# m-schuetz/SimLOD

Hardware: AMD Instinct MI355X
Metric: M points/sec inserted into octree (raster M samples/s @1080p under 'raster') (higher is better)
Workload: dtype f32+u32 (fp32 quantise/project, fp64 pixel coordinate, integer octree/atomics); 1 GPU; Morro Bay 36M stand-in (BASELINE config 2): 36000000 16 B points, fractal terrain, 36 x 1M ring batches resident in HBM, reset + 2.0 kernel_construct launches per step; raster 1920x1080; points_per_gpu=36000000, record_order=shuffled, parallelism=one global cube, level-3 cells dealt to 1 rank(s) by point count

## Files before the change

### simlod_amd/csrc/construct.hip

```cpp
#include <mutex>
#include "simlod_device.hpp"
#include "simlod_hip.h"
#include "simlod_internal.hpp"

namespace simlod {
namespace build {

#include "construct_state.inc"
#include "construct_begin.inc"
#include "construct_count.inc"
#include "construct_expand.inc"
#include "construct_voxelize.inc"
#include "construct_insert.inc"

static_assert(offsetof(Ctl, groupMax) == 44 && offsetof(Ctl, expandNs) + 4 * sizeof(uint64_t) == 184, "Ctl.groupMax at byte 44, Ctl.expandNs[4] at byte 184");

static inline uint64_t align_up(uint64_t v, uint64_t a) { return (v + a - 1) / a * a; }

static constexpr uint64_t ACCT_SPILL_FLOOR = 3500000;
bool layout_construct(BuildArgs& a, uint64_t capacity, bool coalesce, uint32_t groupLimit = SIMLOD_MAX_BATCHES_PER_LAUNCH, uint32_t exactGroup = 1) {
	a.dirCap = 2 * a.nodeCapacity + 65536;
	a.acct = exactGroup > 1u ? 1u : 0u;
	uint64_t off = 4096;
	a.offQueue = off;    off += align_up((uint64_t)CHUNK_QUEUE_CAPACITY * 8, 256);
	a.offSlots = off;    off += align_up((uint64_t)2 * SLOT_CAP * sizeof(SlotRec), 256);
	a.offHist = off;     off += align_up(((uint64_t)SLOT_CAP * HIST_BINS + HIST_EXTRA_WORDS) * 4, 256);
	a.offMap = off;      off += align_up((uint64_t)SLOT_CAP * HIST_BINS * 4, 256);
	a.offHistB = off;    off += align_up((uint64_t)(a.acct ? SLOT_CAP : 0u) * HIST_BINS * exactGroup * 4, 256);
	a.clearCap = 65536;
	a.offClear = off;    off += align_up((uint64_t)2 * a.clearCap * 8, 256);
	a.offTouched = off;  off += align_up((uint64_t)a.nodeCapacity * 4, 256);
	a.crossCap = 16384;
	a.offCross = off;    off += align_up((uint64_t)a.crossCap * 4, 256);
	a.offSplitTag = off; off += align_up((uint64_t)a.nodeCapacity * 8, 256);
	a.offRetryTag = off; off += align_up((uint64_t)a.nodeCapacity * 4, 256);
	a.offTouchTag = off; off += align_up((uint64_t)a.nodeCapacity * 4, 256);
	a.offStartOf = off;  off += align_up((uint64_t)a.nodeCapacity * 8, 256);
	a.offCntB = off;     off += align_up((uint64_t)(a.acct ? a.nodeCapacity : 0u) * exactGroup * 4, 256);
	a.hashCap = 1u << 17;
	a.offHashDir = off;  off += align_up((uint64_t)a.hashCap * sizeof(DirEntry), 256);
	a.offParent = off;   off += align_up((uint64_t)a.nodeCapacity * 4, 256);
	a.offNodeDir = off;  off += align_up((uint64_t)a.nodeCapacity * sizeof(NodeDir), 256);
	a.offChunkDir = off; off += align_up(2ull * a.dirCap * 8, 256);
	a.offLeafChunks = off; off += (uint64_t)a.nodeCapacity * LEAF_ROW_BYTES;
	a.offPaths = off; off += align_up((uint64_t)a.nodeCapacity * PATH_WORDS * 8, 256);
	a.offTop = off;   off += align_up((uint64_t)TOP_CELLS * 4, 256);
	a.offKid = off;   off += align_up((uint64_t)a.nodeCapacity * 4, 256);
	a.voxItemCap = min(a.nodeCapacity + 2u * VOX_BIG_ITEMS, 1u << 20);
	a.offVoxItems = off; off += align_up(2ull * a.voxItemCap * sizeof(VoxItem), 256);
	const uint64_t perBatch = (uint64_t)SIMLOD_MAX_BATCH_SIZE * 4;
	const uint64_t fixedWork = ((uint64_t)SPILLING_CAPACITY + a.nodeCapacity / 8) * 32;
	a.groupMax = 1; a.groupCap = SIMLOD_MAX_BATCH_SIZE;
	if (capacity < off + 2 * perBatch + fixedWork + 4096 + 25ull * 65536) { a.spilledCap = 0; a.scratchBytes = off + 2 * perBatch + fixedWork; return false; }
	const uint64_t freeBytes = capacity - off - fixedWork - 4096;
	if (coalesce) a.groupMax = (uint32_t)std::max<uint64_t>(1, std::min<uint64_t>(std::min<uint32_t>(groupLimit, SIMLOD_MAX_BATCHES_PER_LAUNCH), freeBytes / (2 * perBatch + 20ull * SIMLOD_MAX_BATCH_SIZE)));
	if (a.acct) {
		if (freeBytes < 2ull * exactGroup * perBatch + 512 + ACCT_SPILL_FLOOR * 20032 / 1000) return false;
		a.groupMax = exactGroup;
	}
	a.groupCap = a.groupMax * SIMLOD_MAX_BATCH_SIZE;
	uint64_t cap = (freeBytes - 2ull * a.groupMax * perBatch - 512) * 1000 / (20 * 1000 + 32);
	if (cap > 0x7fffffffull - a.groupCap) cap = 0x7fffffffull - a.groupCap;
	a.spilledCap = (uint32_t)cap;
	a.workCap = a.spilledCap / SIMLOD_POINTS_PER_CHUNK + a.nodeCapacity / 8 + SPILLING_CAPACITY;
	a.offWork = off;     off += align_up((uint64_t)a.workCap * 32, 256);
	a.leafOfStride = align_up((uint64_t)a.groupCap * 4, 256) / 4;
	a.offLeafOf = off;   off += 2 * a.leafOfStride * 4 + align_up((uint64_t)a.spilledCap * 4, 256);
	a.offSpilled = off;  off += (uint64_t)a.spilledCap * 16;
	a.scratchBytes = off;
	return off <= capacity;
}

}
struct SideStream {
	hipStream_t stream;
	hipEvent_t expanded[SIMLOD_MAX_BATCHES_PER_LAUNCH], inserted[SIMLOD_MAX_BATCHES_PER_LAUNCH], tailDone;
	std::mutex enqueue;
};
// ... 139 lines not shown
```

### simlod_amd/csrc/construct_begin.inc

```

__device__ __forceinline__ bool stamp_is_stale(const BuildArgs& a, const Ctl* ctl) {
	const uint32_t first = a.stats->batchletIndex;
	return ctl->tableMagic != TABLE_MAGIC || ctl->tableBatch != first || ctl->tableNodes != (uint64_t)a.nodes || ctl->tablePers != (uint64_t)a.pers ||
	       ctl->tableLayout != layout_signature(a) || ctl->tableSig != table_signature(a.stats) ||
	       (first >= 0x80000u && (first & 0x7ffffu) < SIMLOD_MAX_BATCHES_PER_LAUNCH);
}

__device__ __forceinline__ SimlodChunk*& tail_of(SimlodChunk* head) { return *reinterpret_cast<SimlodChunk**>(&head->size); }

__device__ void rebuild_side_tables(const BuildArgs& a, bool irregular) {
	const uint64_t first = (uint64_t)blockIdx.x * TPB + threadIdx.x, stride = (uint64_t)gridDim.x * TPB;
	{
		uint4* w = reinterpret_cast<uint4*>(a.mom + a.offSplitTag);
		const uint64_t n = (a.offParent - a.offSplitTag) / 16;
		for (uint64_t i = first; i < n; i += stride) w[i] = make_uint4(0, 0, 0, 0);
	}
	const uint32_t numNodes = min(a.stats->numNodes, a.nodeCapacity);
	uint32_t* parentOf = at<uint32_t>(a, a.offParent);
	for (uint64_t i = first; i < TOP_CELLS; i += stride) {
		const uint32_t s = (uint32_t)SIMLOD_MAX_DEPTH - TOP_LEVEL;
		const uint32_t X = ((uint32_t)i >> (2u * TOP_LEVEL)) << s, Y = (((uint32_t)i >> TOP_LEVEL) & (TOP_SIDE - 1u)) << s, Z = ((uint32_t)i & (TOP_SIDE - 1u)) << s;
		uint32_t cur = 0, level = 0;
		while (level < TOP_LEVEL) {
			const SimlodNode* c = a.nodes[cur].children[child_index(X, Y, Z, (int)level)];
// ... 11 lines not shown
			if (c != nullptr) parentOf[(uint32_t)(c - a.nodes)] = (uint32_t)i;
		}
		{
			const SimlodNode* c0 = n->children[0];
			uint32_t word = 0u, some = 0u;
			bool regular = c0 != nullptr;
#pragma unroll
			for (int k = 0; k < 8; k++) {
				const SimlodNode* c = n->children[k];
				if (c != nullptr) some++;
				if (c == nullptr || c != c0 + k) regular = false;
				else if (node_is_leaf(c)) word |= 1u << (KID_LEAF_SHIFT + (uint32_t)k);
			}
			at<uint32_t>(a, a.offKid)[i] = some == 0u ? 0u : regular && !irregular ? (word | (uint32_t)(c0 - a.nodes)) : KID_IRREGULAR;
		}
		uint8_t* const table = a.mom + a.offLeafChunks;
		const bool leaf = node_is_leaf(n);
		SimlodChunk* const head = leaf ? n->points : n->voxelChunks;
		const uint32_t inList = ((leaf ? n->numPoints : n->numVoxelsStored) + SIMLOD_POINTS_PER_CHUNK - 1) / SIMLOD_POINTS_PER_CHUNK;
		SimlodChunk* c = head;
		for (uint32_t k = 0; c != nullptr && k < max(inList, 1u); k++) {
			if (k < LEAF_SLOTS) leaf_row_set(table, a.pers, i, k, c);
			if (k + 1u == inList) tail_of(head) = c;
			c = c->next;
		}
		if (leaf && n->voxelChunks != nullptr) {
			const uint32_t inVox = (n->numVoxelsStored + SIMLOD_POINTS_PER_CHUNK - 1) / SIMLOD_POINTS_PER_CHUNK;
			SimlodChunk* v = n->voxelChunks;
			for (uint32_t k = 0; v != nullptr && k < max(inVox, 1u); k++) {
				if (k + 1u >= inVox) { tail_of(n->voxelChunks) = v; break; }
				v = v->next;
			}
		}
		unsigned long long* rec = at<unsigned long long>(a, a.offPaths) + i * PATH_WORDS;
		const uint32_t L = min(n->level, PATH_WORDS - 1u), s = (uint32_t)SIMLOD_MAX_DEPTH - L;
		const uint32_t X = n->X << s, Y = n->Y << s, Z = n->Z << s;
		uint32_t cur = 0, l = 0;
		for (; l < L; l++) {
			const SimlodNode* anc = a.nodes + cur;
			rec[L - 1u - l] = path_pack(a.pers, cur, anc->level, anc->grid);
			const SimlodNode* c = anc->children[child_index(X, Y, Z, (int)l)];
			if (c == nullptr) break;
			cur = (uint32_t)(c - a.nodes);
		}
		rec[L] = 0;
	}
}

__global__ __launch_bounds__(TPB) void k_begin(BuildArgs a, uint32_t momentaryTooSmall, uint32_t batchLimit, uint32_t debugFlags, uint32_t budgetUs, uint32_t groupMax) {
	Ctl* ctl = ctl_of(a);
	const bool stale = momentaryTooSmall != 0u || (debugFlags & 4u) != 0u || stamp_is_stale(a, ctl);
	if (threadIdx.x == 0 && blockIdx.x == 0) {
		const uint32_t fatal = a.stats->dbg & (SIMLOD_ERR_BARRIER_TIMEOUT | SIMLOD_ERR_DIRECTORY_FULL | SIMLOD_ERR_IMPORT | SIMLOD_ERR_IMPORT_GRID);
		ctl->errors = momentaryTooSmall ? SIMLOD_ERR_MOMENTARY_TOO_SMALL : 0u;
		ctl->stop = (momentaryTooSmall || fatal) ? 1u : 0u;
		ctl->abortBatch = 0;
		ctl->processed = 0;
		ctl->consumed = 0;
		ctl->pointsTaken = a.stats->numPointsProcessed;
		ctl->groupMax = groupMax;
		ctl->debugFlags = debugFlags;
		ctl->budgetUs = budgetUs != 0u ? budgetUs : (uint32_t)(SIMLOD_MAX_PROCESSING_MS * 1000.0f);
		ctl->startNs = wall_ns();
		*a.frameStart = ctl->startNs;
		const uint32_t uploaded = __hip_atomic_load(a.numBatchesUploaded, __ATOMIC_RELAXED, __HIP_MEMORY_SCOPE_AGENT);
		const uint32_t first = a.stats->batchletIndex;
		uint32_t n = uploaded - first;
		if ((int32_t)n < 0) n = 0;
		if (n > SIMLOD_MAX_BATCHES_PER_LAUNCH) n = SIMLOD_MAX_BATCHES_PER_LAUNCH;
		if (n > batchLimit) n = batchLimit;
		ctl->uploaded = uploaded;
		ctl->firstBatch = first;
		ctl->numBatches = n;
		for (int i = 0; i < 8; i++) ctl->statCounters[i] = 0;
		ctl->rebuildLeafChunks = stale ? 1u : 0u;
		if (momentaryTooSmall != 0u) ctl->tableMagic = 0;
		for (uint32_t i = 0; i < BATCH_COPIES; i++) ctl->batch[i].active = 0;
		for (uint32_t i = 0; i < SIMLOD_MAX_BATCHES_PER_LAUNCH; i++) { ctl->voxT[i][0] = ~0ull; ctl->voxT[i][1] = 0; ctl->voxT[i][2] = 0; }
// ... 5 lines not shown
```

### simlod_amd/csrc/construct_expand.inc

```

static constexpr uint32_t VTPB = 1024;
#ifndef VOX_SPT_N
#define VOX_SPT_N 8
#endif
static constexpr uint32_t VOX_SPT = VOX_SPT_N;
static constexpr uint32_t VOX_PIECE = VTPB * VOX_SPT;
static constexpr uint32_t VOX_BIG_ITEMS = 65536;
static constexpr uint32_t VOX_SMALL = 512;
static constexpr uint32_t VOX_SMALL_PIECE = 128;
static constexpr uint32_t LDS_LEVELS = 7;
static constexpr uint32_t CUBE_WORDS = 8192 + 1024 + 256 + 64 + 16 + 4 + 4;
struct VoxItem { uint32_t leaf, s0, s1, ptBase, ptFirst; };
__device__ __forceinline__ VoxItem* vox_items(const BuildArgs& a, const BatchCtl* bc) { return at<VoxItem>(a, a.offVoxItems) + (uint64_t)(bc->ordinal & 1u) * a.voxItemCap; }

#ifndef ALLOC_WAVES_N
#define ALLOC_WAVES_N 10
#endif
static constexpr uint32_t ALLOC_WAVES = ALLOC_WAVES_N, ALLOC_LEAVES = 64 * ALLOC_WAVES;
struct AllocRec {
	uint32_t node, existing, additional, fromPool;
	uint32_t dirNew, prefix;
	unsigned long long firstIdx, mem;
	SimlodChunk* head; SimlodChunk* tail;
};
// ... 373 lines not shown
			}
		}
		if (histHere) {
			__syncthreads();
			for (uint32_t e = threadIdx.x; e < HT_CAP; e += ETPB) {
				const uint32_t key = sh.keys[e];
				if (key != TBL_EMPTY) hist_flush(a, key, sh.vals[e], acct);
			}
			if (timer) { t1 = wall_ns(); ctl->expandNs[0] += t1 - t0; t0 = t1; }
			if (!grid_barrier(&bc->barrierCount, generation, gridDim.x)) { if (threadIdx.x == 0) panic(ctl, SIMLOD_ERR_BARRIER_TIMEOUT); return; }
			if (timer) { t1 = wall_ns(); ctl->expandNs[1] += t1 - t0; t0 = t1; }
		}

		Phase pd(ctl, blockIdx.x == 0);
		for (uint32_t s = sb + blockIdx.x; s < se; s += gridDim.x) {
			uint32_t t = threadIdx.x;
			asm volatile("" : "+v"(t));
			uint64_t before[6] = {0, 0, 0, 0, 0, 0};
			if (pd.on) for (uint32_t k = 0; k < 6u; k++) before[k] = ctl->phaseNs[32u + k];
			const uint32_t myBin = t < HIST_BINS ? hist_sum(hist, (uint64_t)s * HIST_BINS + t) : 0u;
			const SlotRec rec = slots[s];
			if (rec.node == NONE) { if (t == 0u) atomicAdd(&bc->decided, 1u); continue; }
			const uint32_t L = rec.node, l = rec.level;
			const uint32_t K = min(3u, (uint32_t)SIMLOD_MAX_DEPTH - l);
			__syncthreads();
			uint32_t* const B3 = sh.keys; uint32_t* const B2 = B3 + HIST_BINS * GBS; uint32_t* const B1 = B2 + 64u * GBS;
			uint32_t binTotal = myBin;
			if (acct && t < HIST_BINS) {
				const uint32_t* hb = at<const uint32_t>(a, a.offHistB) + ((uint64_t)s * HIST_BINS + t) * GBS;
				for (uint32_t k = 0; k < GB; k++) { const uint32_t r = hb[k]; B3[t * GBS + k] = r; binTotal += r; }
			}
			if (t < HIST_BINS) sh.bins[t] = binTotal;
			if (t < SIMLOD_MAX_BATCHES_PER_LAUNCH) { sh.accD[t] = 0; sh.accF[t] = 0; }
			if (t < PATH_WORDS) sh.pathL[t] = t + 1 < PATH_WORDS ? paths[(uint64_t)L * PATH_WORDS + t] : 0ull;
			if (t == 64u) { const SimlodNode* nl = a.nodes + L; sh.LX = nl->X; sh.LY = nl->Y; sh.LZ = nl->Z; sh.gridL = nl->grid; }
			if (t >= 96u && t < 116u) sh.nameL[t - 96u] = a.nodes[L].name[t - 96u];
			for (uint32_t i = t; i < LOCAL_NODES; i += ETPB) sh.listed[i] = NONE;
			if (t < 72u) sh.grid[t] = nullptr;
			if (t == 0u) { sh.numFresh = 0; sh.numFill = 0; }
			__syncthreads();
			if (t < 64u) { uint32_t c = 0; for (uint32_t k = 0; k < 8; k++) c += sh.bins[t * 8 + k]; sh.c2[t] = c; }
			__syncthreads();
			if (t < 8u) { uint32_t c = 0; for (uint32_t k = 0; k < 8; k++) c += sh.c2[t * 8 + k]; sh.c1[t] = c; }
			__syncthreads();
			if (t < 64u) {
				bool f1 = false, f2 = false;
				if (trunk_any(a) && l + 1u < TRUNK_LEVELS) {
					const uint32_t LX = sh.LX, LY = sh.LY, LZ = sh.LZ, j = t >> 3, k = t & 7u;
					f1 = t < 8u && trunk_forced(a, l + 1u, 2u * LX + ((t >> 2) & 1u), 2u * LY + ((t >> 1) & 1u), 2u * LZ + (t & 1u));
					f2 = trunk_forced(a, l + 2u, 4u * LX + 2u * ((j >> 2) & 1u) + ((k >> 2) & 1u), 4u * LY + 2u * ((j >> 1) & 1u) + ((k >> 1) & 1u), 4u * LZ + 2u * (j & 1u) + (k & 1u));
				}
				{ const unsigned long long bf1 = __ballot(f1), bf2 = __ballot(f2); if (t == 0u) { sh.forced1 = (uint32_t)bf1 & 0xffu; sh.forced2 = bf2; } }
				const bool s1 = t < 8u && K >= 2u && (sh.c1[t & 7u] > SIMLOD_MAX_POINTS_PER_NODE || f1);
				uint32_t mask1 = (uint32_t)__ballot(s1) & 0xffu;
				const bool s2 = K >= 3u && ((mask1 >> (t >> 3)) & 1u) != 0u && (sh.c2[t] > SIMLOD_MAX_POINTS_PER_NODE || f2);
				unsigned long long mask2 = __ballot(s2);
				uint32_t n1 = (uint32_t)__popc(mask1), n2 = (uint32_t)__popcll(mask2);
				uint32_t extraBase = 0, granted = n1 + n2;
				if (t == 0 && n1 + n2 > 0u) {
					uint32_t noSlot, noSpill;
					if (!reserve(a, ctl, bc, 0u, 8u * (n1 + n2), 0u, noSlot, extraBase, noSpill)) {
						const uint32_t inUse = (uint32_t)(__hip_atomic_load(&bc->reserve, __ATOMIC_RELAXED, __HIP_MEMORY_SCOPE_AGENT) >> 32) & 0xfffffu;
						granted = a.nodeCapacity > inUse ? min((a.nodeCapacity - inUse) / 8u, n1 + n2) : 0u;
						if (granted == 0u || !reserve(a, ctl, bc, 0u, 8u * granted, 0u, noSlot, extraBase, noSpill)) { granted = 0u; extraBase = NONE; }
					}
				}
				extraBase = __shfl(extraBase, 0); granted = __shfl(granted, 0);
// ... 146 lines not shown
				uint32_t oct[3] = {0, 0, 0};
				for (uint32_t k = 0; k < depth; k++) oct[k] = (rel >> (3u * (depth - 1u - k))) & 7u;
				uint32_t X = sh.LX, Y = sh.LY, Z = sh.LZ;
				for (uint32_t k = 0; k < depth; k++) { X = 2u * X + ((oct[k] >> 2) & 1u); Y = 2u * Y + ((oct[k] >> 1) & 1u); Z = 2u * Z + (oct[k] & 1u); }
				const bool split = splits(t);
				const bool nextRound = sh.listed[t] != NONE;
				SimlodNode& c = a.nodes[idx];
				const uint32_t firstChild = !split ? 0u : t < 8u ? sh.base2[t] : sh.base3[t - 8u];
				for (uint32_t k = 0; k < 8; k++) c.children[k] = split ? a.nodes + firstChild + k : nullptr;
				kidOf[idx] = !split ? 0u : irregularKids ? KID_IRREGULAR : firstChild | ((t < 8u ? ~(uint32_t)(mask2 >> (8u * t)) & 0xffu : 0xffu) << KID_LEAF_SHIFT);
				uint32_t counter = countOf(t);
				if (acct) {
					if (depth == 3u) {
						const uint32_t born = sh.splitAt[8u + ((t - 72u) >> 3)];
						uint32_t cThen = 0;
						const uint32_t at = nextRound ? split_time(t, born, false, cThen) : NEVER;
						sh.splitAt[t] = (uint8_t)at; sh.counterAt[t] = cThen;
						leaf_chunks(t, born, at);
					}
					if (sh.splitAt[t] != NEVER) counter = sh.counterAt[t];
				}
				c.counter = counter; c.numPoints = 0;
				c.level = level; c.X = X; c.Y = Y; c.Z = Z;
				c.countIteration = 0; c.countFlag = 0;
				for (int k = 0; k < 20; k++) c.name[k] = sh.nameL[k];
				for (uint32_t k = 0; k < depth; k++) if (l + 1u + k < 20u) c.name[l + 1u + k] = (uint8_t)('0' + oct[k]);
				c.visible = 0; c.isFiltered = 0; c.isLeaf = 1; c.isLarge = 0;
				c.grid = split ? sh.grid[t] : nullptr; c.points = nullptr; c.voxelChunks = nullptr;
				c.numVoxels = 0; c.numVoxelsStored = 0;
				if (nextRound) c.grid = grid_of_many(sh.gridMem, numSplit + wantRank);
				const uint32_t parentLocal = depth == 1u ? NONE : depth == 2u ? (t - 8u) >> 3 : 8u + ((t - 72u) >> 3);
				const uint32_t parentIdx = depth == 1u ? L : indexOf(parentLocal);
				parentOf[idx] = parentIdx;
				unsigned long long* mine = paths + (uint64_t)idx * PATH_WORDS;
				uint32_t w = 0;
				if (depth >= 3u) { const uint32_t g = 8u + ((t - 72u) >> 3); mine[w++] = path_pack(a.pers, indexOf(g), l + 2u, sh.grid[g]); }
				if (depth >= 2u) { const uint32_t ch = depth == 2u ? (t - 8u) >> 3 : (t - 72u) >> 6; mine[w++] = path_pack(a.pers, indexOf(ch), l + 1u, sh.grid[ch]); }
				mine[w++] = path_pack(a.pers, L, l, sh.gridL);
				for (uint32_t k = 0; w < PATH_WORDS; k++) {
					const unsigned long long e = w + 1 < PATH_WORDS ? sh.pathL[k] : 0ull;
					mine[w++] = e;
					if (e == 0ull) break;
				}
				if (t < 8u) a.nodes[L].children[t] = a.nodes + idx;
				if (!split && countOf(t) != 0u && !nextRound) sh.fresh[atomicAdd(&sh.numFresh, 1u)] = FreshLeaf{idx, countOf(t), level, X, Y, Z};
				if (level <= TOP_LEVEL && (!split || level == TOP_LEVEL)) {
					const uint32_t mark = split ? 0u : TOP_LEAF;
					if (TOP_LEVEL - level <= 1u) top_fill(at<uint32_t>(a, a.offTop), idx, level, X, Y, Z, mark);
					else sh.fill[atomicAdd(&sh.numFill, 1u)] = make_uint4(idx | (level << 19) | mark, X, Y, Z);
				}
			}
			if (t == 0u) {
				kidOf[L] = irregularKids ? KID_IRREGULAR : rec.childBase | ((~mask1 & 0xffu) << KID_LEAF_SHIFT);
				if (L != 0u) {
					const uint32_t P = parentOf[L];
					if (P != NONE && kidOf[P] != KID_IRREGULAR) atomicAnd(&kidOf[P], ~(1u << (KID_LEAF_SHIFT + octant_of(sh.LX, sh.LY, sh.LZ))));
				}
				if (l == TOP_LEVEL) at<uint32_t>(a, a.offTop)[(sh.LX << (2u * TOP_LEVEL)) | (sh.LY << TOP_LEVEL) | sh.LZ] = L | (l << 19);
				a.nodes[L].numPoints = 0; a.nodes[L].points = nullptr;
				if (acct && rec.born == NONE) a.nodes[L].counter = sh.counterAt[LOCAL_NODES];
			}
			if (t < HIST_BINS) {
				const uint32_t j = t >> 6, jk = t >> 3;
				const uint32_t u = ((mask1 >> j) & 1u) == 0u ? j : ((mask2 >> jk) & 1ull) == 0ull ? 8u + jk : 72u + t;
				const uint32_t ls = sh.listed[u];
				map[(uint64_t)s * HIST_BINS + t] = ls != NONE ? ls : indexOf(u);
			}
			__syncthreads();
			pd.mark(35);
			if (acct && t < GB) {
				if (sh.accD[t] != 0u) atomicAdd(&bc->acctD[t], sh.accD[t]);
				if (sh.accF[t] != 0u) atomicAdd(&bc->acctF[t], sh.accF[t]);
			}
// ... 126 lines not shown
```

### simlod_amd/csrc/construct_state.inc

```

static constexpr uint32_t SLOT_CAP_GRIDS = 256;
static constexpr uint32_t BATCH_COPIES = 4;
struct BatchCtl {
	uint32_t active, batchSize, ringSlot, batchIndex;
	uint32_t ordinal, tag, slotsRound0, numSpilled;
	uint32_t numWork, numClear, numTouched, numCross;
	uint32_t barrierCount, rootPieces, numVoxItems, numVoxSmall;
	uint32_t groupBatches, dirCount, acct, accounted;
	uint32_t start[SIMLOD_MAX_BATCHES_PER_LAUNCH + 1];
	uint32_t slot[SIMLOD_MAX_BATCHES_PER_LAUNCH];
	uint32_t decided;
	unsigned long long reserve;
	unsigned long long reserve0;
	uint32_t acctAlloc0, acctPool0, rootSplitAt, pad5;
	uint32_t acctD[SIMLOD_MAX_BATCHES_PER_LAUNCH], acctF[SIMLOD_MAX_BATCHES_PER_LAUNCH];
};

struct Ctl {
	uint32_t uploaded, firstBatch, numBatches, stop;
	uint32_t errors, abortBatch, rebuildLeafChunks, debugFlags;
	uint32_t processed, budgetUs, consumed, groupMax;
	uint64_t startNs;
	uint32_t statCounters[8];
	uint32_t tableMagic, tableBatch;
// ... 95 lines not shown
}
template <uint32_t REP>
__device__ __forceinline__ uint32_t spread_sum(const SpreadTable<REP>& t, uint32_t e) {
	uint32_t s = 0;
#pragma unroll
	for (uint32_t r = 0; r < REP; r++) s += t.vals[e * REP + r];
	return s;
}

__device__ __forceinline__ int table_find(const BlockTable& t, uint32_t key) {
	uint32_t h = table_hash(key);
#pragma unroll 1
	for (int probe = 0; probe < 16; ++probe) {
		const uint32_t k = t.keys[h];
		if (k == key) return (int)h;
		if (k == TBL_EMPTY) return -1;
		h = (h + 1) & (TBL_CAP - 1);
	}
	return -1;
}



static constexpr uint32_t TPB = 256;

struct NodeDir {
	uint32_t ptBase, ptFirst, ptTag, pad0;
};

static constexpr uint32_t LEAF_SLOTS = LEAF_ROW_SLOTS;
static constexpr uint32_t TABLE_MAGIC = 0x51ab1e05u;
static_assert(LEAF_SLOTS <= 64, "queue_split hands a leaf's chunks out one per lane");

static constexpr uint32_t PATH_WORDS = SIMLOD_MAX_DEPTH + 1;
static constexpr unsigned long long PATH_VALID = 1ull << 63;

__device__ __forceinline__ unsigned long long path_pack(const uint8_t* pers, uint32_t nodeIdx, uint32_t level, const SimlodOccupancyGrid* grid) {
	const unsigned long long off = (unsigned long long)(reinterpret_cast<const uint8_t*>(grid) - pers) >> 4;
	return PATH_VALID | ((unsigned long long)nodeIdx << 41) | ((unsigned long long)level << 36) | off;
}
__device__ __forceinline__ uint32_t path_node(unsigned long long e) { return (uint32_t)(e >> 41) & 0x7ffffu; }
__device__ __forceinline__ uint32_t path_level(unsigned long long e) { return (uint32_t)(e >> 36) & 31u; }
__device__ __forceinline__ SimlodOccupancyGrid* path_grid(uint8_t* pers, unsigned long long e) {
	return reinterpret_cast<SimlodOccupancyGrid*>(pers + ((e & 0xfffffffffull) << 4));
}

static constexpr uint32_t TOP_LEVEL = 5, TOP_SIDE = 1u << TOP_LEVEL, TOP_CELLS = TOP_SIDE * TOP_SIDE * TOP_SIDE;
__device__ __forceinline__ uint32_t top_cell(uint32_t X, uint32_t Y, uint32_t Z) {
	const uint32_t s = (uint32_t)SIMLOD_MAX_DEPTH - TOP_LEVEL;
	return (((X >> s) & (TOP_SIDE - 1u)) << (2u * TOP_LEVEL)) | (((Y >> s) & (TOP_SIDE - 1u)) << TOP_LEVEL) | ((Z >> s) & (TOP_SIDE - 1u));
}
__device__ __forceinline__ void top_fill(uint32_t* top, uint32_t idx, uint32_t level, uint32_t X, uint32_t Y, uint32_t Z, uint32_t mark) {
	const uint32_t k = TOP_LEVEL - level, side = 1u << k, x0 = X << k, y0 = Y << k, z0 = Z << k, e = idx | (level << 19) | mark;
	for (uint32_t i = 0; i < (1u << (3u * k)); i++) {
		const uint32_t dx = i >> (2u * k), dy = (i >> k) & (side - 1u), dz = i & (side - 1u);
		top[((x0 + dx) << (2u * TOP_LEVEL)) | ((y0 + dy) << TOP_LEVEL) | (z0 + dz)] = e;
	}
}

static constexpr uint32_t KID_IRREGULAR = 0xffffffffu, KID_LEAF_SHIFT = 19, TOP_LEAF = 0x80000000u;
__device__ __forceinline__ uint32_t octant_of(uint32_t X, uint32_t Y, uint32_t Z) { return ((X & 1u) << 2) | ((Y & 1u) << 1) | (Z & 1u); }

__device__ __forceinline__ Ctl* ctl_of(const BuildArgs& a) { return reinterpret_cast<Ctl*>(a.mom); }
template <class T> __device__ __forceinline__ T* at(const BuildArgs& a, uint64_t off) { return reinterpret_cast<T*>(a.mom + off); }

__device__ __forceinline__ BatchCtl* batch_of(Ctl* ctl, uint32_t ordinal) {
	BatchCtl* bc = &ctl->batch[ordinal % BATCH_COPIES];
	return bc->active != 0u && bc->ordinal == ordinal ? bc : nullptr;
}

struct Phase {
	Ctl* ctl; bool on; uint64_t t;
	__device__ __forceinline__ Phase(Ctl* c, bool who) : ctl(c), on(SIMLOD_MEASURE != 0 && who && threadIdx.x == 0), t(on ? wall_ns() : 0) {}
	__device__ __forceinline__ void mark(uint32_t k) { if (on) { const uint64_t n = wall_ns(); ctl->phaseNs[k] += n - t; t = n; } }
};

struct VoxItem;
// ... 64 lines not shown
	bc->dirCount = 0;
	bc->reserve = 0;
	bc->acct = a.acct != 0u && take > 1u ? 1u : 0u;
	bc->accounted = 0;
	bc->rootSplitAt = 0xffffffffu;
	for (uint32_t k = 0; k < SIMLOD_MAX_BATCHES_PER_LAUNCH; k++) { bc->acctD[k] = 0; bc->acctF[k] = 0; }
	bc->active = 1;
}

template <bool SINGLE>
struct Samples {
	const float4* ring; const float4* only; const BatchCtl* bc; uint32_t batches;
	__device__ __forceinline__ Samples(const BuildArgs& a, const BatchCtl* b) : ring(reinterpret_cast<const float4*>(a.ring)), bc(b), batches(b->groupBatches) {
		only = ring + (size_t)b->ringSlot * SIMLOD_MAX_BATCH_SIZE;
	}
	__device__ __forceinline__ const float4* ptr(uint32_t i) const {
		if (SINGLE || batches == 1u) return only + i;
		uint32_t k = min(i / SIMLOD_MAX_BATCH_SIZE, batches - 1u);
		while (k + 1u < batches && i >= bc->start[k + 1u]) k++;
		return ring + (size_t)bc->slot[k] * SIMLOD_MAX_BATCH_SIZE + (i - bc->start[k]);
	}
	__device__ __forceinline__ float4 operator[](uint32_t i) const { return *ptr(i); }
	__device__ __forceinline__ bool span(uint32_t i0, uint32_t i1, const float4*& base, uint32_t& k) const {
		k = 0; base = only;
		if (SINGLE || batches == 1u) return true;
		k = min(i0 / SIMLOD_MAX_BATCH_SIZE, batches - 1u);
		while (k + 1u < batches && i0 >= bc->start[k + 1u]) k++;
		base = ring + (size_t)bc->slot[k] * SIMLOD_MAX_BATCH_SIZE - bc->start[k];
		return i1 < bc->start[k + 1u];
	}
};

__host__ __device__ inline uint64_t layout_signature(const BuildArgs& a) {
	return a.scratchBytes ^ ((uint64_t)a.nodeCapacity << 40) ^ ((uint64_t)a.groupMax << 59) ^ (a.offSpilled * 0x9E3779B97F4A7C15ull);
}
```

### simlod_amd/csrc/construct_voxelize.inc

```

struct DirEntry { unsigned long long key; SimlodChunk* ptr; };
static constexpr unsigned long long DIR_BUSY = 1ull << 62;
__device__ __forceinline__ unsigned long long dir_key(uint32_t tag, uint32_t node, uint32_t k) {
	return (1ull << 63) | ((unsigned long long)(tag & 0xfffffu) << 42) | ((unsigned long long)node << 22) | (k & 0x3fffffu);
}
__device__ __forceinline__ uint32_t dir_tag(unsigned long long key) { return (uint32_t)(key >> 42) & 0xfffffu; }
__device__ __forceinline__ uint32_t dir_hash(const BuildArgs& a, unsigned long long key) {
	key ^= key >> 29; key *= 0x9e3779b97f4a7c15ull; key ^= key >> 32;
	return (uint32_t)key & (a.hashCap - 1u);
}
__device__ __forceinline__ unsigned long long ld_agent(const unsigned long long* p) { return __hip_atomic_load(p, __ATOMIC_RELAXED, __HIP_MEMORY_SCOPE_AGENT); }

__device__ void dir_insert(const BuildArgs& a, Ctl* ctl, uint32_t tag, uint32_t node, uint32_t k, SimlodChunk* c) {
	DirEntry* dir = at<DirEntry>(a, a.offHashDir);
	const unsigned long long key = dir_key(tag, node, k);
	uint32_t h = dir_hash(a, key);
	for (uint32_t probe = 0; probe < a.hashCap; probe++, h = (h + 1u) & (a.hashCap - 1u)) {
		unsigned long long cur = ld_agent(&dir[h].key);
		while (cur == 0ull || ((cur >> 63) != 0ull && dir_tag(cur) != (tag & 0xfffffu))) {
			const unsigned long long prev = atomicCAS(&dir[h].key, cur, DIR_BUSY);
			if (prev == cur) {
				__hip_atomic_store(reinterpret_cast<unsigned long long*>(&dir[h].ptr), (unsigned long long)c, __ATOMIC_RELAXED, __HIP_MEMORY_SCOPE_AGENT);
				asm volatile("s_waitcnt vmcnt(0)" ::: "memory");
				__hip_atomic_store(&dir[h].key, key, __ATOMIC_RELAXED, __HIP_MEMORY_SCOPE_AGENT);
// ... 92 lines not shown
	const uint32_t rel = w - cube_offset(d), row = d == 1u ? rel >> 1 : rel, ly = row % side, lz = row / side;
	const uint32_t cell = ox + 128u * (oy + ly) + 16384u * (oz + lz);
	gridWord = (cell >> 5) + (d == 1u ? (rel & 1u) : 0u);
	shift = d <= 2u ? 0u : (cell & 31u);
	mask = side >= 32u ? 0xffffffffu : (1u << side) - 1u;
	return d;
}

__device__ __forceinline__ void voxelize_small(const BuildArgs& a, Ctl* ctl, BatchCtl* bc, const uint32_t wave, const uint32_t numWaves) {
	const uint32_t numSmall = min(bc->numVoxSmall, a.voxItemCap - VOX_BIG_ITEMS);
	if (numSmall == 0u) return;
	const VoxItem* items = vox_items(a, bc);
	SimlodChunk* const* chunkDir = chunk_dir(a, bc);
	const uint32_t tag = bc->tag;
	const uint32_t lane = (uint32_t)lane_id();
	constexpr uint32_t U = 4;
	const uint32_t per = numSmall > numWaves / 4u ? U : 1u;
	for (uint32_t k0 = wave * per; k0 < numSmall; k0 += numWaves * per) {
		VoxItem it[U];
		unsigned long long mine[U];
		uint32_t itemIndex[U], count[U], depth[U];
		uint32_t maxCount = 0, maxDepth = 0;
#pragma unroll
		for (uint32_t u = 0; u < U; u++) {
			itemIndex[u] = VOX_BIG_ITEMS + min(k0 + u, numSmall - 1u);
			it[u] = items[itemIndex[u]];
		}
#pragma unroll
		for (uint32_t u = 0; u < U; u++) {
			const uint32_t leafIdx = it[u].leaf & 0xffffffu;
			count[u] = u < per && k0 + u < numSmall ? it[u].s1 - it[u].s0 : 0u;
			mine[u] = 0ull;
			if (leafIdx == 0u) { SimlodOccupancyGrid* g = a.nodes[0].grid; if (lane == 0u && g != nullptr) mine[u] = path_pack(a.pers, 0u, 0u, g); }
			else if (lane < PATH_WORDS - 1) mine[u] = (at<const unsigned long long>(a, a.offPaths) + (uint64_t)leafIdx * PATH_WORDS)[lane];
		}
#pragma unroll
		for (uint32_t u = 0; u < U; u++) {
			const unsigned long long present = __ballot(mine[u] != 0ull);
			depth[u] = count[u] != 0u ? (uint32_t)__ffsll((long long)~present) - 1u : 0u;
			maxCount = max(maxCount, count[u]); maxDepth = max(maxDepth, depth[u]);
		}
		for (uint32_t base = 0; base < maxCount; base += 64u) {
			uint32_t pX[U], pY[U], pZ[U];
			float color[U];
			bool go[U];
			{
				float4 p[U];
#pragma unroll
				for (uint32_t u = 0; u < U; u++) {
					const uint32_t rel = base + lane, i = it[u].s0 + rel;
					go[u] = rel < count[u];
					p[u] = go[u] ? reinterpret_cast<const float4*>(chunkDir[it[u].ptBase + (i / SIMLOD_POINTS_PER_CHUNK - it[u].ptFirst)]->points)[i % SIMLOD_POINTS_PER_CHUNK] : make_float4(0, 0, 0, 0);
				}
#pragma unroll
				for (uint32_t u = 0; u < U; u++) {
					pX[u] = quantize(F_FULL, p[u].x, a.minx, a.size); pY[u] = quantize(F_FULL, p[u].y, a.miny, a.size); pZ[u] = quantize(F_FULL, p[u].z, a.minz, a.size);
					color[u] = p[u].w;
				}
			}
			for (uint32_t d = 1; d <= maxDepth; d++) {
				bool any = false;
#pragma unroll
				for (uint32_t u = 0; u < U; u++) { go[u] = go[u] && d <= depth[u]; any = any || go[u]; }
				if (__ballot(any) == 0ull) break;
				unsigned long long ent[U];
				uint32_t* word[U]; uint32_t bit[U], seen[U], level[U];
#pragma unroll
// ... 35 lines not shown
		if (elapsedMs > (float)ctl->budgetUs / 1000.0f) __hip_atomic_store(&ctl->stop, 1u, __ATOMIC_RELAXED, __HIP_MEMORY_SCOPE_AGENT);
	}
}

static constexpr uint32_t VOXROOT_WGS = 8;
__device__ __forceinline__ void voxroot_pieces(const BuildArgs& a, Ctl* ctl, BatchCtl* bc, VoxShared& sh, uint32_t wg, uint32_t numWgs);

__global__ __launch_bounds__(VTPB) void k_voxelize(BuildArgs a, uint32_t ordinal) {
	Ctl* ctl = ctl_of(a);
	BatchCtl* bc = batch_of(ctl, ordinal);
	if (bc == nullptr || ctl->abortBatch) return;
	__shared__ VoxShared sh;
	const uint32_t numWgs = gridDim.x - VOXROOT_WGS;
	if (blockIdx.x >= numWgs) {
		if (bc->rootPieces != 0u) voxroot_pieces(a, ctl, bc, sh, blockIdx.x - numWgs, VOXROOT_WGS);
		return;
	}
	if (blockIdx.x == 0 && threadIdx.x == 0) end_of_batch(a, ctl, bc);
	const uint32_t numItems = min(bc->numVoxItems, VOX_BIG_ITEMS);
	const VoxItem* items = vox_items(a, bc);
	SimlodChunk* const* chunkDir = chunk_dir(a, bc);
	const uint32_t tag = bc->tag;
	static_assert(VTPB == 1024 && CUBE_WORDS <= 9216 + VTPB, "k_voxelize: thread t owns the LDS cube words t + 1024 k (k < 8: cube 1), 8192 + t (cube 2), 9216 + t (cubes 3..7)");
	const uint32_t lane = (uint32_t)lane_id();
	Phase ph(ctl, blockIdx.x == ((ctl->debugFlags >> 8) & 0xffffu));
	const bool clocked = SIMLOD_MEASURE != 0 && (ctl->debugFlags & 2u) != 0u;
	if (clocked && blockIdx.x == 0 && threadIdx.x == 0) ctl->voxT[ordinal][0] = wall_ns();
	for (uint32_t item = blockIdx.x; item < numItems; item += numWgs) {
		VoxItem it = items[item];
		const uint32_t leafLevel = it.leaf >> 24;
		it.leaf &= 0xffffffu;
		if (it.leaf == 0u) continue;
		const uint32_t LX = a.nodes[it.leaf].X, LY = a.nodes[it.leaf].Y, LZ = a.nodes[it.leaf].Z;
		const unsigned long long* rec = at<const unsigned long long>(a, a.offPaths) + (uint64_t)it.leaf * PATH_WORDS;
		__syncthreads();
		if (threadIdx.x < PATH_WORDS) {
			const unsigned long long e = threadIdx.x < PATH_WORDS - 1 ? rec[threadIdx.x] : 0ull;
			sh.anc[threadIdx.x] = e; sh.cnt[threadIdx.x] = 0; sh.hiOcc[threadIdx.x] = 0; sh.hiFresh[threadIdx.x] = 0; sh.rank[threadIdx.x] = 0;
			if (threadIdx.x < 8u) sh.listCount[threadIdx.x] = 0;
		}
		const SimlodChunk* chunk[VOX_SPT];
		bool live[VOX_SPT];
#pragma unroll
		for (uint32_t j = 0; j < VOX_SPT; j++) {
			const uint32_t i = it.s0 + j * VTPB + threadIdx.x;
			live[j] = i < it.s1;
			chunk[j] = live[j] ? chunkDir[it.ptBase + (i / SIMLOD_POINTS_PER_CHUNK - it.ptFirst)] : nullptr;
		}
		__syncthreads();
		ph.mark(24);
		uint32_t depth = 0;
		while (depth < PATH_WORDS - 1 && sh.anc[depth] != 0ull) depth++;
		const uint32_t ldsDepth = min(depth, LDS_LEVELS);

		const uint32_t g1 = ((((LX & 1u) * 64u) + 128u * ((LY & 1u) * 64u) + 16384u * ((LZ & 1u) * 64u)) >> 5) + ((threadIdx.x >> 1) & 63u) * 4u + (threadIdx.x >> 7) * 512u + (threadIdx.x & 1u);
		const uint32_t g2 = (((LX & 3u) * 32u) + 128u * ((LY & 3u) * 32u + (threadIdx.x & 31u)) + 16384u * ((LZ & 3u) * 32u + (threadIdx.x >> 5))) >> 5;
		const uint32_t w3 = 9216u + threadIdx.x;
		uint32_t gw3, sft3, msk3;
		const uint32_t d3 = cube_word(w3, LX, LY, LZ, gw3, sft3, msk3);
		const bool have3 = d3 != 0u && d3 <= ldsDepth;
		uint32_t* const grid1 = ldsDepth >= 1u ? path_grid(a.pers, sh.anc[0])->values : nullptr;
		uint32_t* const grid2 = ldsDepth >= 2u ? path_grid(a.pers, sh.anc[1])->values : nullptr;
		uint32_t* const grid3 = have3 ? path_grid(a.pers, sh.anc[d3 - 1u])->values : nullptr;
		uint32_t snap1[8], snap2, snap3;
		{
#pragma unroll
			for (uint32_t k = 0; k < 8; k++) snap1[k] = ldsDepth >= 1u ? grid1[g1 + k * 4096u] : 0u;
			snap2 = ldsDepth >= 2u ? grid2[g2] : 0u;
			snap3 = have3 ? grid3[gw3] : 0u;
			uint32_t hi = 0;
// ... 248 lines not shown
```

Before: 15280 M points/s.

## Truncate per-node ancestor path rows and chain to ancestors for deep levels

Per-node ancestor path records shrink from PATH_WORDS (max depth + 1) entries to a fixed PATH_ROW of 12 entries. Entries deeper than that are found by following the last stored ancestor's row (path_far). This cuts the scratch footprint and the write traffic for path rows in rebuild and expand, and makes rows fit tighter in cache. In exchange, leaves deeper than 12 levels need dependent chained loads, and the layout signature now includes the row size.

```diff
diff --git a/simlod_amd/csrc/construct.hip b/simlod_amd/csrc/construct.hip
--- a/simlod_amd/csrc/construct.hip
+++ b/simlod_amd/csrc/construct.hip
@@ -43,7 +43,7 @@
 	a.offNodeDir = off;  off += align_up((uint64_t)a.nodeCapacity * sizeof(NodeDir), 256);
 	a.offChunkDir = off; off += align_up(2ull * a.dirCap * 8, 256);
 	a.offLeafChunks = off; off += (uint64_t)a.nodeCapacity * LEAF_ROW_BYTES;
-	a.offPaths = off; off += align_up((uint64_t)a.nodeCapacity * PATH_WORDS * 8, 256);
+	a.offPaths = off; off += align_up((uint64_t)a.nodeCapacity * PATH_ROW * 8, 256);
 	a.offTop = off;   off += align_up((uint64_t)TOP_CELLS * 4, 256);
 	a.offKid = off;   off += align_up((uint64_t)a.nodeCapacity * 4, 256);
 	a.voxItemCap = min(a.nodeCapacity + 2u * VOX_BIG_ITEMS, 1u << 20);
diff --git a/simlod_amd/csrc/construct_begin.inc b/simlod_amd/csrc/construct_begin.inc
--- a/simlod_amd/csrc/construct_begin.inc
+++ b/simlod_amd/csrc/construct_begin.inc
@@ -67,18 +67,18 @@
 				v = v->next;
 			}
 		}
-		unsigned long long* rec = at<unsigned long long>(a, a.offPaths) + i * PATH_WORDS;
+		unsigned long long* rec = at<unsigned long long>(a, a.offPaths) + i * PATH_ROW;
 		const uint32_t L = min(n->level, PATH_WORDS - 1u), s = (uint32_t)SIMLOD_MAX_DEPTH - L;
 		const uint32_t X = n->X << s, Y = n->Y << s, Z = n->Z << s;
 		uint32_t cur = 0, l = 0;
 		for (; l < L; l++) {
 			const SimlodNode* anc = a.nodes + cur;
-			rec[L - 1u - l] = path_pack(a.pers, cur, anc->level, anc->grid);
+			if (L - 1u - l < PATH_ROW) rec[L - 1u - l] = path_pack(a.pers, cur, anc->level, anc->grid);
 			const SimlodNode* c = anc->children[child_index(X, Y, Z, (int)l)];
 			if (c == nullptr) break;
 			cur = (uint32_t)(c - a.nodes);
 		}
-		rec[L] = 0;
+		if (L < PATH_ROW) rec[L] = 0;
 	}
 }
 
diff --git a/simlod_amd/csrc/construct_expand.inc b/simlod_amd/csrc/construct_expand.inc
--- a/simlod_amd/csrc/construct_expand.inc
+++ b/simlod_amd/csrc/construct_expand.inc
@@ -429,7 +429,11 @@
 			}
 			if (t < HIST_BINS) sh.bins[t] = binTotal;
 			if (t < SIMLOD_MAX_BATCHES_PER_LAUNCH) { sh.accD[t] = 0; sh.accF[t] = 0; }
-			if (t < PATH_WORDS) sh.pathL[t] = t + 1 < PATH_WORDS ? paths[(uint64_t)L * PATH_WORDS + t] : 0ull;
+			if (t < PATH_WORDS) {
+				unsigned long long e = t < PATH_ROW ? paths[(uint64_t)L * PATH_ROW + t] : 0ull;
+				if (t >= PATH_ROW && t < l) e = path_far(paths, L, t, a.nodeCapacity);
+				sh.pathL[t] = e;
+			}
 			if (t == 64u) { const SimlodNode* nl = a.nodes + L; sh.LX = nl->X; sh.LY = nl->Y; sh.LZ = nl->Z; sh.gridL = nl->grid; }
 			if (t >= 96u && t < 116u) sh.nameL[t - 96u] = a.nodes[L].name[t - 96u];
 			for (uint32_t i = t; i < LOCAL_NODES; i += ETPB) sh.listed[i] = NONE;
@@ -642,13 +646,13 @@
 				const uint32_t parentLocal = depth == 1u ? NONE : depth == 2u ? (t - 8u) >> 3 : 8u + ((t - 72u) >> 3);
 				const uint32_t parentIdx = depth == 1u ? L : indexOf(parentLocal);
 				parentOf[idx] = parentIdx;
-				unsigned long long* mine = paths + (uint64_t)idx * PATH_WORDS;
+				unsigned long long* mine = paths + (uint64_t)idx * PATH_ROW;
 				uint32_t w = 0;
 				if (depth >= 3u) { const uint32_t g = 8u + ((t - 72u) >> 3); mine[w++] = path_pack(a.pers, indexOf(g), l + 2u, sh.grid[g]); }
 				if (depth >= 2u) { const uint32_t ch = depth == 2u ? (t - 8u) >> 3 : (t - 72u) >> 6; mine[w++] = path_pack(a.pers, indexOf(ch), l + 1u, sh.grid[ch]); }
 				mine[w++] = path_pack(a.pers, L, l, sh.gridL);
-				for (uint32_t k = 0; w < PATH_WORDS; k++) {
-					const unsigned long long e = w + 1 < PATH_WORDS ? sh.pathL[k] : 0ull;
+				for (uint32_t k = 0; w < PATH_ROW; k++) {
+					const unsigned long long e = sh.pathL[k];
 					mine[w++] = e;
 					if (e == 0ull) break;
 				}
diff --git a/simlod_amd/csrc/construct_state.inc b/simlod_amd/csrc/construct_state.inc
--- a/simlod_amd/csrc/construct_state.inc
+++ b/simlod_amd/csrc/construct_state.inc
@@ -151,7 +151,12 @@
 static constexpr uint32_t TABLE_MAGIC = 0x51ab1e05u;
 static_assert(LEAF_SLOTS <= 64, "queue_split hands a leaf's chunks out one per lane");
 
+#ifndef PATH_DIRECT
+#define PATH_DIRECT 12
+#endif
 static constexpr uint32_t PATH_WORDS = SIMLOD_MAX_DEPTH + 1;
+static constexpr uint32_t PATH_ROW = PATH_DIRECT;
+static_assert(PATH_ROW >= 3u && PATH_ROW <= (uint32_t)SIMLOD_MAX_DEPTH, "k_expand writes up to three entries of a new node's row before it copies the slot node's path");
 static constexpr unsigned long long PATH_VALID = 1ull << 63;
 
 __device__ __forceinline__ unsigned long long path_pack(const uint8_t* pers, uint32_t nodeIdx, uint32_t level, const SimlodOccupancyGrid* grid) {
@@ -162,6 +167,14 @@
 __device__ __forceinline__ uint32_t path_level(unsigned long long e) { return (uint32_t)(e >> 36) & 31u; }
 __device__ __forceinline__ SimlodOccupancyGrid* path_grid(uint8_t* pers, unsigned long long e) {
 	return reinterpret_cast<SimlodOccupancyGrid*>(pers + ((e & 0xfffffffffull) << 4));
+}
+__device__ inline unsigned long long path_far(const unsigned long long* paths, uint32_t node, uint32_t k, uint32_t nodeCapacity) {
+	while (k >= PATH_ROW) {
+		const unsigned long long last = paths[(uint64_t)node * PATH_ROW + (PATH_ROW - 1u)];
+		node = path_node(last); k -= PATH_ROW;
+		if (last == 0ull || node >= nodeCapacity) return 0ull;
+	}
+	return paths[(uint64_t)node * PATH_ROW + k];
 }
 
 static constexpr uint32_t TOP_LEVEL = 5, TOP_SIDE = 1u << TOP_LEVEL, TOP_CELLS = TOP_SIDE * TOP_SIDE * TOP_SIDE;
@@ -292,5 +305,5 @@
 };
 
 __host__ __device__ inline uint64_t layout_signature(const BuildArgs& a) {
-	return a.scratchBytes ^ ((uint64_t)a.nodeCapacity << 40) ^ ((uint64_t)a.groupMax << 59) ^ (a.offSpilled * 0x9E3779B97F4A7C15ull);
-}
+	return a.scratchBytes ^ ((uint64_t)a.nodeCapacity << 40) ^ ((uint64_t)a.groupMax << 59) ^ (a.offSpilled * 0x9E3779B97F4A7C15ull) ^ ((uint64_t)PATH_ROW * 0xC2B2AE3D27D4EB4Full);
+}
diff --git a/simlod_amd/csrc/construct_voxelize.inc b/simlod_amd/csrc/construct_voxelize.inc
--- a/simlod_amd/csrc/construct_voxelize.inc
+++ b/simlod_amd/csrc/construct_voxelize.inc
@@ -148,7 +148,11 @@
 			count[u] = u < per && k0 + u < numSmall ? it[u].s1 - it[u].s0 : 0u;
 			mine[u] = 0ull;
 			if (leafIdx == 0u) { SimlodOccupancyGrid* g = a.nodes[0].grid; if (lane == 0u && g != nullptr) mine[u] = path_pack(a.pers, 0u, 0u, g); }
-			else if (lane < PATH_WORDS - 1) mine[u] = (at<const unsigned long long>(a, a.offPaths) + (uint64_t)leafIdx * PATH_WORDS)[lane];
+			else {
+				const unsigned long long* paths = at<const unsigned long long>(a, a.offPaths);
+				if (lane < PATH_ROW) mine[u] = paths[(uint64_t)leafIdx * PATH_ROW + lane];
+				if ((it[u].leaf >> 24) > PATH_ROW && lane >= PATH_ROW && lane < (it[u].leaf >> 24)) mine[u] = path_far(paths, leafIdx, lane, a.nodeCapacity);
+			}
 		}
 #pragma unroll
 		for (uint32_t u = 0; u < U; u++) {
@@ -250,10 +254,11 @@
 		it.leaf &= 0xffffffu;
 		if (it.leaf == 0u) continue;
 		const uint32_t LX = a.nodes[it.leaf].X, LY = a.nodes[it.leaf].Y, LZ = a.nodes[it.leaf].Z;
-		const unsigned long long* rec = at<const unsigned long long>(a, a.offPaths) + (uint64_t)it.leaf * PATH_WORDS;
+		const unsigned long long* rec = at<const unsigned long long>(a, a.offPaths) + (uint64_t)it.leaf * PATH_ROW;
 		__syncthreads();
 		if (threadIdx.x < PATH_WORDS) {
-			const unsigned long long e = threadIdx.x < PATH_WORDS - 1 ? rec[threadIdx.x] : 0ull;
+			unsigned long long e = threadIdx.x < PATH_ROW ? rec[threadIdx.x] : 0ull;
+			if (leafLevel > PATH_ROW && threadIdx.x >= PATH_ROW && threadIdx.x < leafLevel) e = path_far(at<const unsigned long long>(a, a.offPaths), it.leaf, threadIdx.x, a.nodeCapacity);
 			sh.anc[threadIdx.x] = e; sh.cnt[threadIdx.x] = 0; sh.hiOcc[threadIdx.x] = 0; sh.hiFresh[threadIdx.x] = 0; sh.rank[threadIdx.x] = 0;
 			if (threadIdx.x < 8u) sh.listCount[threadIdx.x] = 0;
 		}
```

Result: faster. 15720 M points/s, median of 6 (+2.9%).
